# lhwright13/Hybrid-Classical-and-Reinforcement-Learning-Aircraft-Controllers

Hardware: AMD Instinct MI355X
Metric: env-steps/sec (whole node), rate-control task, batch 65536 per GPU (higher is better)
Workload: dtype f32 compute / f64 state

## Files before the change

hybrid-classical-and-reinforcement-learning-aircraft-controllers_amd/csrc/fdyn_kernels.hip:

```cpp
#include <hip/hip_runtime.h>
#include <stdint.h>
#include <math.h>
#include <string.h>
#include <stdlib.h>
#include "fdyn_core.hpp"
#include "../../include/fdyn.h"

using namespace fdyn;

#define FD_BLOCK 256
#define FD_MAX_TYPES 8
#define FD_WAVE 64

template <typename T>
__device__ __forceinline__ void stage(T* dst, const T* __restrict__ src, int n)
{
    for (int i = threadIdx.x; i < n; i += blockDim.x) dst[i] = src[i];
}

template <bool FAST>
__device__ __forceinline__ void stage_params(double* s_params, const double* __restrict__ params, int n_types)
{
    for (int i = threadIdx.x; i < n_types * FD_NP_USED; i += blockDim.x) {
        const int t = i / FD_NP_USED, k = i - t * FD_NP_USED;
// ... 443 lines not shown
            if (idx >= n_wp) { if (restart) idx = 0; else frozen = true; }
            if (!frozen) surf = waypoint_agent<G>(cfg, st, Cr, s_wps + idx * FD_NWP, xg, derive(), gdt, inner);
            return;
        }
        const G c0 = G(cmd[i]), c1 = G(cmd[n + i]), c2 = G(cmd[2 * n + i]), c3 = G(cmd[3 * n + i]);
        if (level == FD_LEVEL_ATTITUDE) {
            const bool has_yaw = c2 == c2;
            surf = attitude_agent<G>(cfg, st, Cr, c0, c1, has_yaw ? c2 : G(0), has_yaw, c3, xg, gdt, inner);
        } else if (level == FD_LEVEL_HSA) {
            surf = hsa_agent<G>(cfg, st, Cr, c0, c1, c2, xg, derive(), gdt, inner);
        } else {
            const G wp[FD_NWP] = { c0, c1, c2, c3 };
            surf = waypoint_agent<G>(cfg, st, Cr, wp, xg, derive(), gdt, inner);
        }
    };
    if constexpr (FAST) {
        FastRK f;
        f.init(x);
        outer(f.x0, [&]() { return derived_fast(f); });
    } else {
        outer(x, [&]() { return derived<S>(x); });
    }

#pragma unroll
    for (int k = 0; k < FD_NX; ++k) if (actions) xs[k * n + i] = x[k];
#pragma unroll
    for (int k = 0; k < FD_NPID; ++k) {
        pid_state[(k * FD_NPS + FD_PS_INTEGRAL) * n + i] = st[k].integral;
        pid_state[(k * FD_NPS + FD_PS_ERR_PREV) * n + i] = st[k].err_prev;
        pid_state[(k * FD_NPS + FD_PS_DFILT) * n + i] = st[k].dfilt;
    }
    if (mission) {
        wp_idx[i] = idx;
        if (reached_total) reached_total[i] += reached;
    }
    if (is_pid) {
        surf_out[FD_U_ELEVATOR * n + i] = S(surf.elevator); surf_out[FD_U_AILERON * n + i] = S(surf.aileron);
        surf_out[FD_U_RUDDER * n + i] = S(surf.rudder);
    } else if (actions) {
        surf_out[FD_U_ELEVATOR * n + i] = S(applied.elevator); surf_out[FD_U_AILERON * n + i] = S(applied.aileron);
        surf_out[FD_U_RUDDER * n + i] = S(applied.rudder);
    }
    surf_out[FD_U_THROTTLE * n + i] = S(surf.throttle);
    const float rc[4] = { float(inner.p), float(inner.q), float(inner.r), float(inner.thr) };
    if (rate_cmd_out) {
#pragma unroll
        for (int k = 0; k < 4; ++k) rate_cmd_out[k * n + i] = rc[k];
    }
    {
#pragma clang fp contract(off)
        float* o = obs_out + i * FD_OBS_DIM;
        const double mr[3] = { consts[FD_C_MAX_ROLL_RATE], consts[FD_C_MAX_PITCH_RATE], consts[FD_C_MAX_YAW_RATE] };
#pragma unroll
        for (int k = 0; k < 3; ++k) {
            const S c = clipv(S(rc[k]), -S(mr[k]), S(mr[k]));
            o[k] = float(x[9 + k]);
            o[3 + k] = float(c);
            o[6 + k] = float(c - x[9 + k]);
        }
        o[9] = float(M<S>::sqrt(x[3] * x[3] + x[4] * x[4] + x[5] * x[5]));
        o[10] = float(-x[2]);
        o[11] = float(x[6]); o[12] = float(x[7]); o[13] = float(x[8]);
#pragma unroll
        for (int k = 0; k < FD_ACT_DIM; ++k) o[14 + k] = pa[k];
    }
}

template <typename G> struct EnvConsts {
    G dt, mr0, mr1, mr2, scale;
    int max_steps, cmd_type, n_sub;
    int settle_steps;
    __device__ __forceinline__ G max_rate(int ax) const { return mr0 * G(ax == 0) + mr1 * G(ax == 1) + mr2 * G(ax == 2); }
};

template <typename G>
__device__ __forceinline__ void env_load(EnvState<G>& e, const G* __restrict__ es, int64_t n, int64_t i, bool sched = true)
{
#pragma unroll
    for (int k = 0; k < 3; ++k) {
        e.cmd[k] = es[(FD_E_CMD_P + k) * n + i];
        e.prev_err[k] = es[(FD_E_PERR_P + k) * n + i];
        e.sign_changes[k] = es[(FD_E_SIGN_P + k) * n + i];
    }
#pragma unroll
    for (int k = 0; k < 4; ++k) {
        e.prev_action[k] = es[(FD_E_PREV_AIL + k) * n + i];
        e.sched[k] = sched ? es[(FD_E_SCHED0 + k) * n + i] : G(0);
    }
    e.settle_timer = es[FD_E_SETTLE_TIMER * n + i]; e.is_settled = es[FD_E_IS_SETTLED * n + i];
    e.time = es[FD_E_TIME * n + i]; e.ep_return = es[FD_E_EP_RETURN * n + i];
}
template <typename G>
__device__ __forceinline__ void env_store(const EnvState<G>& e, G* __restrict__ es, int64_t n, int64_t i, bool sched = true)
{
#pragma unroll
    for (int k = 0; k < 3; ++k) {
        es[(FD_E_CMD_P + k) * n + i] = e.cmd[k];
        es[(FD_E_PERR_P + k) * n + i] = e.prev_err[k];
        es[(FD_E_SIGN_P + k) * n + i] = e.sign_changes[k];
    }
#pragma unroll
    for (int k = 0; k < 4; ++k) {
        es[(FD_E_PREV_AIL + k) * n + i] = e.prev_action[k];
        if (sched) es[(FD_E_SCHED0 + k) * n + i] = e.sched[k];
    }
    es[FD_E_SETTLE_TIMER * n + i] = e.settle_timer; es[FD_E_IS_SETTLED * n + i] = e.is_settled;
    es[FD_E_TIME * n + i] = e.time; es[FD_E_EP_RETURN * n + i] = e.ep_return;
}

template <typename G>
__device__ __forceinline__ void device_reset_record(uint64_t seed, uint32_t env, uint32_t episode,
                                                    const EnvConsts<G>& ec, G (&rec)[FD_NR])
{
    Philox ph;
    uint32_t r0[4], r1[4], r2[4], r3[4];
    ph.block(seed, env, episode, 0u, FD_PHX_RESET + 0, r0);
    ph.block(seed, env, episode, 0u, FD_PHX_RESET + 1, r1);
    ph.block(seed, env, episode, 0u, FD_PHX_RESET + 2, r2);
    ph.block(seed, env, episode, 0u, FD_PHX_RESET + 3, r3);
    const float d15 = 0.26179938779914943f;
    rec[FD_R_AIRSPEED] = G(15.0f + 15.0f * u01(r0[0]));
    rec[FD_R_ALTITUDE] = G(50.0f + 150.0f * u01(r0[1]));
    rec[FD_R_ROLL] = G(-d15 + 2.0f * d15 * u01(r0[2]));
    rec[FD_R_PITCH] = G(-d15 + 2.0f * d15 * u01(r0[3]));
    rec[FD_R_YAW] = G(6.283185307179586f * u01(r1[0]));
    rec[FD_R_P] = G(-0.1f + 0.2f * u01(r1[1]));
    rec[FD_R_Q] = G(-0.1f + 0.2f * u01(r1[2]));
    rec[FD_R_R] = G(-0.1f + 0.2f * u01(r1[3]));
    rec[FD_R_CMD0] = rec[FD_R_CMD1] = rec[FD_R_CMD2] = rec[FD_R_CMD3] = G(0);
    if (ec.cmd_type == FD_CMD_RANDOM_WALK) return;
    const bool sine = ec.cmd_type == FD_CMD_SINE;
    int k = sine ? 1 + int(u01(r2[0]) * 2.0f) : 1 + int(u01(r2[0]) * 3.0f);
    k = k > 3 ? 3 : k;
    const int perm = int(u01(r2[1]) * 6.0f) % 6;
    const int first = perm >> 1;
    const int o1 = first == 2 ? 0 : first + 1, o2 = first == 0 ? 2 : first - 1;
    const int second = (perm & 1) ? o2 : o1;
    const float m0 = u01(r3[0]), m1 = u01(r3[1]), m2 = u01(r3[2]);
    const G mrs[3] = { ec.mr0, ec.mr1, ec.mr2 };
    G vals[3];
#pragma unroll
    for (int a = 0; a < 3; ++a) {
        const int pos = (a == first) ? 0 : ((a == second) ? 1 : 2);
        const float um = pos == 0 ? m0 : (pos == 1 ? m1 : m2);
        float mag = (0.3f + 0.7f * um) * float(ec.scale);
        if (sine) mag *= 0.5f;
        const float sgn = (!sine && ((r2[2] >> pos) & 1u)) ? -1.0f : 1.0f;
        vals[a] = (pos < k) ? G(sgn * mag) * mrs[a] : G(0);
    }
    rec[FD_R_CMD0] = vals[0]; rec[FD_R_CMD1] = vals[1]; rec[FD_R_CMD2] = vals[2];
    if (sine) rec[FD_R_CMD3] = G(0.1f + 1.9f * u01(r2[3]));
}

template <typename G, typename E>
__device__ __forceinline__ void env_apply_reset(const G (&rec)[FD_NR], int cmd_type, G (&x)[FD_NX], EnvState<E>& e)
{
#pragma unroll
    for (int k = 0; k < FD_NX; ++k) x[k] = G(0);
    x[2] = -rec[FD_R_ALTITUDE]; x[3] = rec[FD_R_AIRSPEED];
    x[6] = rec[FD_R_ROLL]; x[7] = rec[FD_R_PITCH]; x[8] = rec[FD_R_YAW];
    x[9] = rec[FD_R_P]; x[10] = rec[FD_R_Q]; x[11] = rec[FD_R_R];
#pragma unroll
    for (int k = 0; k < 3; ++k) { e.cmd[k] = E(0); e.prev_err[k] = E(0); e.sign_changes[k] = E(0); e.prev_action[k] = E(0); }
#pragma unroll
    for (int k = 0; k < 4; ++k) e.sched[k] = E(0);
    e.prev_action[3] = E(0.5);
    if (cmd_type == FD_CMD_STEP) {
        e.cmd[0] = E(rec[FD_R_CMD0]); e.cmd[1] = E(rec[FD_R_CMD1]); e.cmd[2] = E(rec[FD_R_CMD2]);
    } else if (cmd_type == FD_CMD_RAMP || cmd_type == FD_CMD_SINE) {
        e.sched[0] = E(rec[FD_R_CMD0]); e.sched[1] = E(rec[FD_R_CMD1]); e.sched[2] = E(rec[FD_R_CMD2]); e.sched[3] = E(rec[FD_R_CMD3]);
    }
    e.settle_timer = E(0); e.is_settled = E(0); e.time = E(0); e.ep_return = E(0);
}

template <typename G, bool PREP = false>
__device__ __forceinline__ void load_env_consts(const double* __restrict__ EC, EnvConsts<G>& ec)
{
    ec.dt = G(EC[FD_EC_DT]);
    if constexpr (!PREP) {
        ec.max_steps = int(EC[FD_EC_MAX_STEPS]);
        ec.cmd_type = int(EC[FD_EC_CMD_TYPE]);
    }
    ec.scale = G(EC[FD_EC_DIFFICULTY_SCALE]);
    ec.mr0 = G(EC[FD_EC_MAX_RATE_P]); ec.mr1 = G(EC[FD_EC_MAX_RATE_Q]); ec.mr2 = G(EC[FD_EC_MAX_RATE_R]);
    if constexpr (PREP) {
        const int32_t* __restrict__ ic = reinterpret_cast<const int32_t*>(EC + FD_ECD_INTS);
        ec.max_steps = ic[0]; ec.cmd_type = ic[1]; ec.n_sub = ic[2]; ec.settle_steps = ic[3];
        return;
    }
    const double r = EC[FD_EC_DT] / EC[FD_EC_DT_PHYSICS];
    const long ns = long(r);
    ec.n_sub = ns < 1 ? 1 : int(ns);
    const double dts = EC[FD_EC_DT];
    int k = 0;
    if (dts >= 1.0e-3) { double t = 0.0; while (t < 0.2 && k < 256) { t += dts; ++k; } }
    else k = int(0.2 / dts) + 1;
    ec.settle_steps = k;
}

template <typename G>
__device__ __forceinline__ void fetch_reset_record(const double* __restrict__ pool, int pool_depth, uint64_t seed,
                                                   int64_t i, int32_t episode, const EnvConsts<G>& ec, G (&rec)[FD_NR])
{
    if (pool) {
        const double* r = pool + (i * pool_depth + (episode % pool_depth)) * FD_NR;
#pragma unroll
        for (int k = 0; k < FD_NR; ++k) rec[k] = G(r[k]);
#pragma unroll
        for (int k = 0; k < FD_NR; ++k) asm volatile("" : "+v"(rec[k]));
    } else {
        device_reset_record<G>(seed, uint32_t(i), uint32_t(episode), ec, rec);
    }
}

__device__ __forceinline__ void store_obs_tile(float* tile , const float (&o)[FD_OBS_DIM], int lane,
                                               float* __restrict__ obs_out, int64_t wave_first, int64_t n)
{
    int64_t valid = n - wave_first;
    valid = valid < 0 ? 0 : (valid < FD_WAVE ? valid : FD_WAVE);
    float* dst = obs_out + wave_first * FD_OBS_DIM;
    static_assert(FD_OBS_DIM == 18 && FD_WAVE == 64, "the full-wave path below moves 64 x 18 floats as 288 float4");
    if (valid == FD_WAVE && (reinterpret_cast<uintptr_t>(dst) & 15) == 0) {
        float2* row = reinterpret_cast<float2*>(tile + lane * FD_OBS_DIM);
#pragma unroll
        for (int k = 0; k < FD_OBS_DIM / 2; ++k) row[k] = make_float2(o[2 * k], o[2 * k + 1]);
        __builtin_amdgcn_wave_barrier();
        const float4* t4 = reinterpret_cast<const float4*>(tile);
        float4* d4 = reinterpret_cast<float4*>(dst);
#pragma unroll
        for (int j = 0; j < 4; ++j) d4[j * FD_WAVE + lane] = t4[j * FD_WAVE + lane];
        if (lane < FD_WAVE / 2) d4[4 * FD_WAVE + lane] = t4[4 * FD_WAVE + lane];
        __builtin_amdgcn_wave_barrier();
        return;
    }
#pragma unroll
    for (int k = 0; k < FD_OBS_DIM; ++k) tile[lane * (FD_OBS_DIM + 1) + k] = o[k];
    __builtin_amdgcn_wave_barrier();
#pragma unroll
    for (int k = 0; k < FD_OBS_DIM; ++k) {
        const int flat = k * FD_WAVE + lane;
        const int row = flat / FD_OBS_DIM, col = flat - row * FD_OBS_DIM;
        if (row < valid) dst[flat] = tile[row * (FD_OBS_DIM + 1) + col];
    }
    __builtin_amdgcn_wave_barrier();
}

template <typename S> __device__ __forceinline__ void dr_unpack(S*& dr, const double*& drc, S* d, const double* c) { dr = d; drc = c; }
__device__ __forceinline__ void dr_normals3(uint64_t seed, uint32_t env, uint32_t episode, uint32_t step, uint32_t word, float (&z)[3])
{
    Philox ph; uint32_t r[4];
    ph.block(seed, env, episode, step, word, r);
    const float m0 = fast::sqrt(-2.0f * __logf(u01(r[0]))), m1 = fast::sqrt(-2.0f * __logf(u01(r[2])));
    float s0, c0, s1, c1;
    fast::sincos(6.283185307179586f * u01(r[1]), s0, c0);
    fast::sincos(6.283185307179586f * u01(r[3]), s1, c1);
    z[0] = m0 * c0; z[1] = m0 * s0; z[2] = m1 * c1;
}
template <typename A, typename S>
__device__ __forceinline__ void air_velocity(const S (&x)[FD_NX], const S (&W)[3], A& ua, A& va, A& wa)
{
    A sp, cp, st, ct, sy, cy, bu, bv, bw;
    M<A>::sincos(A(x[6]), sp, cp); M<A>::sincos(A(x[7]), st, ct); M<A>::sincos(A(x[8]), sy, cy);
    body_wind<A>(sp, cp, st, ct, sy, cy, Wind<A>{ A(W[0]), A(W[1]), A(W[2]) }, bu, bv, bw);
    ua = A(x[3]) - bu; va = A(x[4]) - bv; wa = A(x[5]) - bw;
}
template <typename A, typename S>
__device__ __forceinline__ A air_speed(const S (&x)[FD_NX], const S (&W)[3])
{
    A ua, va, wa;
    air_velocity<A, S>(x, W, ua, va, wa);
    return M<A>::sqrt(ua * ua + va * va + wa * wa);
}
template <typename S>
__device__ __forceinline__ void dr_reset(uint64_t seed, uint32_t env, uint32_t episode, const double* __restrict__ drc, double dt,
                                         S* __restrict__ dr, int64_t n, int64_t i, S (&x)[FD_NX], S (&wair)[3])
{
    if (drc[FD_DC_REDRAW] != 0.0) {
        Philox ph;
        uint32_t r0[4], r1[4], r2[4];
        ph.block(seed, env, episode, 0u, FD_PHX_DR_RESET, r0);
        ph.block(seed, env, episode, 0u, FD_PHX_DR_RESET + 1, r1);
        ph.block(seed, env, episode, 0u, FD_PHX_DR_RESET + 2, r2);
        const uint32_t u[10] = { r0[0], r0[1], r0[2], r0[3], r1[0], r1[1], r1[2], r1[3], r2[0], r2[1] };
        double v[10];
#pragma unroll
        for (int k = 0; k < 10; ++k) {
            const double lo = drc[2 * k], hi = drc[2 * k + 1];
            v[k] = lo + (hi - lo) * double(u01(u[k]));
        }
        float sd, cd;
        fast::sincos(float(v[1]), sd, cd);
        float z[3];
        dr_normals3(seed, env, episode, 0u, FD_PHX_DR_GUST0, z);
        const double V0 = double(x[3]);
        const double sigma = v[3] * V0;
        const double a = exp(-dt * V0 / v[4]);
        const S row[FD_NDR] = { S(v[0] * double(cd)), S(v[0] * double(sd)), S(v[2]),
                                S(sigma * double(z[0])), S(sigma * double(z[1])), S(sigma * double(z[2])),
                                S(a), S(sigma * sqrt(1.0 - a * a)),
                                S(v[5]), S(v[6]), S(v[7]), S(v[8]), S(v[9]) };
#pragma unroll
        for (int k = 0; k < FD_NDR; ++k) dr[k * n + i] = row[k];
#pragma unroll
        for (int k = 0; k < 3; ++k) wair[k] = row[FD_DR_WIND_N + k] + row[FD_DR_GUST_N + k];
    } else {
#pragma unroll
        for (int k = 0; k < 3; ++k) wair[k] = dr[(FD_DR_WIND_N + k) * n + i] + dr[(FD_DR_GUST_N + k) * n + i];
    }
    S sp, cp, st, ct, sy, cy, bu, bv, bw;
    M<S>::sincos(x[6], sp, cp); M<S>::sincos(x[7], st, ct); M<S>::sincos(x[8], sy, cy);
    body_wind<S>(sp, cp, st, ct, sy, cy, Wind<S>{ wair[0], wair[1], wair[2] }, bu, bv, bw);
    x[3] = x[3] + bu; x[4] = x[4] + bv; x[5] = x[5] + bw;
}

template <typename S, typename E, typename... DRA>
__global__ void __launch_bounds__(FD_BLOCK)
rate_env_reset_kernel(S* __restrict__ xs, E* __restrict__ es, int32_t* __restrict__ eis, float* __restrict__ pid_state,
                      const uint8_t* __restrict__ mask, const double* __restrict__ EC, const double* __restrict__ pool,
                      int pool_depth, uint64_t seed, float* __restrict__ obs_out, int64_t n, DRA... dra)
{
    __shared__ __attribute__((aligned(16))) float s_tile[FD_BLOCK / FD_WAVE][FD_WAVE * (FD_OBS_DIM + 1)];
    constexpr bool DR = sizeof...(DRA) != 0;
    S* dr = nullptr;
    const double* drc = nullptr;
    if constexpr (DR) dr_unpack(dr, drc, dra...);
    const LaneMap lm = lane_map(n);
    const int64_t i = lm.i;
    const int lane = lm.lane, wave = threadIdx.x / FD_WAVE;
    const bool active = lm.on;
    EnvConsts<S> ec;
    load_env_consts<S>(EC, ec);
    S x[FD_NX];
    EnvState<E> e;
    float o[FD_OBS_DIM];
#pragma unroll
    for (int k = 0; k < FD_OBS_DIM; ++k) o[k] = 0.0f;
    if (active) {
        const bool doit = mask ? mask[i] != 0 : true;
        S wair[3];
        if (doit) {
            const int32_t episode = eis[FD_EI_EPISODE * n + i];
            S rec[FD_NR];
            fetch_reset_record<S>(pool, pool_depth, seed, i, episode, ec, rec);
            env_apply_reset<S, E>(rec, ec.cmd_type, x, e);
            if constexpr (DR) dr_reset<S>(seed, uint32_t(i), uint32_t(episode), drc, EC[FD_EC_DT], dr, n, i, x, wair);
#pragma unroll
            for (int k = 0; k < FD_NX; ++k) xs[k * n + i] = x[k];
            env_store<E>(e, es, n, i);
            eis[FD_EI_STEP * n + i] = 0;
            eis[FD_EI_EPISODE * n + i] = episode + 1;
            if (pid_state) for (int k = 0; k < 3 * FD_NPS; ++k) pid_state[k * n + i] = 0.0f;
        } else {
#pragma unroll
            for (int k = 0; k < FD_NX; ++k) x[k] = xs[k * n + i];
            env_load<E>(e, es, n, i);
            if constexpr (DR) {
#pragma unroll
                for (int k = 0; k < 3; ++k) wair[k] = dr[(FD_DR_WIND_N + k) * n + i] + dr[(FD_DR_GUST_N + k) * n + i];
            }
        }
        S airspeed, altitude;
        airspeed_altitude<S>(x, airspeed, altitude);
        if constexpr (DR) airspeed = air_speed<S, S>(x, wair);
        env_observation<S, S, E>(x, e, airspeed, altitude, o);
    }
    store_obs_tile(s_tile[wave], o, lane, obs_out, lm.wave_first, n);
}

#ifdef FD_PHASE_STAMPS
__device__ unsigned long long fdyn_stamps[4096 * 8];
#define FD_STAMP(K) if (threadIdx.x == 0 && blockIdx.x < 4096) fdyn_stamps[blockIdx.x * 8 + (K)] = __builtin_readcyclecounter();
#define FD_STAMP_REAL(K) if (threadIdx.x == 0 && blockIdx.x < 4096) fdyn_stamps[blockIdx.x * 8 + (K)] = wall_clock64();
extern "C" int fdyn_debug_read_stamps(unsigned long long* out, int count)
{
    return int(hipMemcpyFromSymbol(out, HIP_SYMBOL(fdyn_stamps), sizeof(unsigned long long) * size_t(count)));
}
extern "C" int fdyn_debug_read_counts(unsigned* out, int count, int clear)
{
    int rc = int(hipMemcpyFromSymbol(out, HIP_SYMBOL(fdyn_dbg_cnt), sizeof(unsigned) * size_t(count)));
    if (clear && rc == 0) {
        void* p = nullptr;
        rc = int(hipGetSymbolAddress(&p, HIP_SYMBOL(fdyn_dbg_cnt)));
        if (rc == 0) rc = int(hipMemset(p, 0, sizeof(unsigned) * 4096 * 8));
    }
    return rc;
}
#else
#define FD_STAMP(K)
#define FD_STAMP_REAL(K)
#endif

template <typename S, typename T, bool OCC2, bool PREP, typename... DRA>
__global__ void __launch_bounds__(FD_BLOCK, OCC2 ? 2 : 1)
rate_env_step_kernel(S* __restrict__ xs, typename EnvOf<S, T>::type* __restrict__ es, int32_t* __restrict__ eis,
                     const uint8_t* __restrict__ type, const double* __restrict__ params, int n_types,
                     const double* __restrict__ EC,
                     const float* __restrict__ actions ,
                     float* __restrict__ pid_state , const float* __restrict__ pid_cfg ,
                     const double* __restrict__ casc_consts , float* __restrict__ actions_out,
                     const S* __restrict__ rw_delta ,
                     const double* __restrict__ pool, int pool_depth, uint64_t seed, int auto_reset, float residual_scale,
                     float* __restrict__ obs_out , float* __restrict__ reward_f32, S* __restrict__ reward_full,
                     uint8_t* __restrict__ terminated, uint8_t* __restrict__ truncated,
                     int32_t* __restrict__ ev_count, int32_t* __restrict__ ev_count_next, int32_t* __restrict__ ev_int,
                     float* __restrict__ ev_flt, int ev_cap, int64_t n, DRA... dra)
{
    constexpr bool DR = sizeof...(DRA) != 0;
    S* dr = nullptr;
    const double* drc = nullptr;
    if constexpr (DR) dr_unpack(dr, drc, dra...);
    __shared__ double s_params[FD_MAX_TYPES * FD_NP_STAGED];
    __shared__ __attribute__((aligned(16))) float s_tile[FD_BLOCK / FD_WAVE][FD_WAVE * (FD_OBS_DIM + 1)];
    __shared__ float s_pid_cfg[3 * FD_NPC];
    __shared__ S s_consts[FD_NC];
    FD_STAMP(0)
    FD_STAMP_REAL(7)
    const LaneMap lm = lane_map(n);
    const int64_t i = lm.i;
    const int lane = lm.lane, wave = threadIdx.x / FD_WAVE;
    const bool active = lm.on;
    EnvConsts<S> ec;
    load_env_consts<S, PREP>(EC, ec);
    const bool uses_sched = ec.cmd_type == FD_CMD_RAMP || ec.cmd_type == FD_CMD_SINE;
    const bool residual_mode = actions != nullptr && residual_scale > 0.0f && pid_state != nullptr;
    const bool pid_mode = actions == nullptr || residual_mode;

    using E = typename EnvOf<S, T>::type;
    S x[FD_NX];
    EnvState<E> e;
    int32_t step = 0, episode = 0;
    int ty = 0;
    float4 av = make_float4(0.0f, 0.0f, 0.0f, 0.0f);
    S rec_pre[FD_NR];
    S wair[3] = { S(0), S(0), S(0) }, dsc[5] = { S(1), S(1), S(1), S(1), S(1) };
    const bool pre_drawn = !OCC2 && pool == nullptr && auto_reset != 0;
    constexpr bool EARLY_PARAMS = sizeof(T) == 4;
    StagedParamWords spw = { 0.0, 0.0, 1.0 };
    if constexpr (EARLY_PARAMS) spw = PREP ? stage_image_early(params, n_types) : stage_params_early(params, n_types);
    if (active) {
        episode = eis[FD_EI_EPISODE * n + i];
#pragma unroll
        for (int k = 3; k < FD_NX; ++k) x[k] = xs[k * n + i];
        if (actions) av = reinterpret_cast<const float4*>(actions)[i];
        ty = lane_type(type, i, n_types);
#pragma unroll
        for (int k = 0; k < 3; ++k) x[k] = xs[k * n + i];
        step = eis[FD_EI_STEP * n + i];
        env_load<E>(e, es, n, i, uses_sched);
        if (pre_drawn) device_reset_record<S>(seed, uint32_t(i), uint32_t(episode), ec, rec_pre);
        if constexpr (DR) {
#pragma unroll
            for (int k = 0; k < 3; ++k) wair[k] = dr[(FD_DR_WIND_N + k) * n + i] + dr[(FD_DR_GUST_N + k) * n + i];
#pragma unroll
            for (int k = 0; k < 5; ++k) dsc[k] = dr[(FD_DR_MASS_S + k) * n + i];
        }
    }
    if constexpr (PREP) {
        if constexpr (EARLY_PARAMS) stage_image_finish(s_params, spw, n_types);
        else stage(s_params, params, n_types * FD_NP_STAGED);
    } else if constexpr (EARLY_PARAMS) stage_params_finish<true>(s_params, spw, n_types);
    else stage_params<false>(s_params, params, n_types);
    if (pid_mode) {
        stage(s_pid_cfg, pid_cfg, 3 * FD_NPC);
        for (int k = threadIdx.x; k < FD_NC; k += blockDim.x) s_consts[k] = S(casc_consts[k]);
    }
    __syncthreads();

    if (ev_count_next && blockIdx.x == 0 && threadIdx.x < FD_EV_SHARDS) ev_count_next[threadIdx.x] = 0;

    float o[FD_OBS_DIM];
#pragma unroll
    for (int k = 0; k < FD_OBS_DIM; ++k) o[k] = 0.0f;
    bool done = false, term = false;
    S reward = S(0);

    if (active) {
        const double* blk = s_params + ty * FD_NP_STAGED;
        Params<T> P; P.load(blk);
        if constexpr (DR) scale_params<T>(P, double(dsc[0]), double(dsc[1]), double(dsc[2]), double(dsc[3]), double(dsc[4]));
        Limits<S> Lm; Lm.load(blk);

        float a_in[4];
        S res_bonus = S(0);
        if (!pid_mode) {
            a_in[0] = av.x; a_in[1] = av.y; a_in[2] = av.z; a_in[3] = av.w;
        } else {
            PidCfg cfg[3]; PidState st[3];
#pragma unroll
            for (int k = 0; k < 3; ++k) {
                cfg[k] = load_pid_cfg(s_pid_cfg, k);
                st[k] = PidState{ pid_state[(k * FD_NPS + 0) * n + i], pid_state[(k * FD_NPS + 1) * n + i], pid_state[(k * FD_NPS + 2) * n + i] };
            }
            const S pid_dt = s_consts[FD_C_PID_DT] > S(0) ? s_consts[FD_C_PID_DT] : ec.dt;
            const Surfaces<S> sf = rate_agent<S>(cfg, st, s_consts, S(e.cmd[0]), S(e.cmd[1]), S(e.cmd[2]), s_consts[FD_C_PID_THROTTLE], x, pid_dt);
            a_in[0] = float(sf.aileron); a_in[1] = float(sf.elevator); a_in[2] = float(sf.rudder); a_in[3] = float(sf.throttle);
#pragma unroll
            for (int k = 0; k < 3; ++k) {
                pid_state[(k * FD_NPS + 0) * n + i] = st[k].integral; pid_state[(k * FD_NPS + 1) * n + i] = st[k].err_prev;
                pid_state[(k * FD_NPS + 2) * n + i] = st[k].dfilt;
            }
            if (residual_mode) {
#pragma clang fp contract(off)
                const float rr[4] = { av.x, av.y, av.z, av.w };
#pragma unroll
                for (int k = 0; k < 4; ++k) {
                    const float c = a_in[k] + rr[k] * residual_scale;
                    const float lo = k < 3 ? -1.0f : 0.0f;
                    a_in[k] = c < lo ? lo : (c > 1.0f ? 1.0f : c);
                }
                const float mag = rr[0] * rr[0] + (rr[1] * rr[1] + rr[2] * rr[2]);
                res_bonus = S(0.05) * (S(1) - S(mag) / S(3));
            }
        }
        if (actions_out) reinterpret_cast<float4*>(actions_out)[i] = make_float4(a_in[0], a_in[1], a_in[2], a_in[3]);
        S a[4];
        a[0] = clipv(S(a_in[0]), S(-1), S(1)); a[1] = clipv(S(a_in[1]), S(-1), S(1));
        a[2] = clipv(S(a_in[2]), S(-1), S(1)); a[3] = clipv(S(a_in[3]), S(0), S(1));

        Controls<T> C;
        C.set(P, a[1], a[0], a[2], a[3]);
        const S dt_sub = ec.dt / S(ec.n_sub);
#ifdef FD_PHASE_STAMPS
        asm volatile("s_waitcnt vmcnt(0) lgkmcnt(0)" ::: "memory");
#endif
        FD_STAMP(1)
        if constexpr (DR) rk4_substeps<S, T, !OCC2, true>(P, Lm, C, x, dt_sub, ec.n_sub, Wind<T>{ T(wair[0]), T(wair[1]), T(wair[2]) });
        else rk4_substeps<S, T, !OCC2>(P, Lm, C, x, dt_sub, ec.n_sub);
        FD_STAMP(2)
        if constexpr (sizeof(E) == sizeof(S)) e.time += E(ec.dt);
        else e.time = E(S(step + 1) * ec.dt);
        step += 1;

        if (ec.cmd_type == FD_CMD_RAMP) {
            const S t = S(e.time);
            if (t < S(3)) {
                const S alpha = t / S(3);
#pragma unroll
                for (int k = 0; k < 3; ++k) e.cmd[k] = E((S(1) - alpha) * S(0) + alpha * S(e.sched[k]));
            } else {
#pragma unroll
                for (int k = 0; k < 3; ++k) e.cmd[k] = e.sched[k];
            }
        } else if (ec.cmd_type == FD_CMD_RANDOM_WALK) {
            S delta[3];
            if (rw_delta) {
#pragma unroll
                for (int k = 0; k < 3; ++k) delta[k] = rw_delta[k * n + i];
            } else {
                Philox ph; uint32_t r[4];
                ph.block(seed, uint32_t(i), uint32_t(episode), uint32_t(step), FD_PHX_RANDOM_WALK, r);
                const float m0 = sqrtf(-2.0f * logf(u01(r[0]))), m1 = sqrtf(-2.0f * logf(u01(r[2])));
                const float n0 = m0 * cosf(6.283185307f * u01(r[1])), n1 = m0 * sinf(6.283185307f * u01(r[1]));
                const float n2 = m1 * cosf(6.283185307f * u01(r[3]));
                const S sd = S(0.1) * M<S>::sqrt(ec.dt) * ec.scale;
                delta[0] = S(n0) * sd * ec.mr0; delta[1] = S(n1) * sd * ec.mr1; delta[2] = S(n2) * sd * ec.mr2;
            }
#pragma unroll
            for (int k = 0; k < 3; ++k) e.cmd[k] = E(clipv(S(e.cmd[k]) + delta[k], -ec.max_rate(k), ec.max_rate(k)));
        } else if (ec.cmd_type == FD_CMD_SINE) {
            const S sn = M<S>::sin(S(2.0 * FD_PI) * S(e.sched[3]) * S(e.time));
#pragma unroll
            for (int k = 0; k < 3; ++k) e.cmd[k] = E(S(e.sched[k]) * sn);
        }

        if constexpr (DR) {
            float z[3];
            dr_normals3(seed, uint32_t(i), uint32_t(episode), uint32_t(step), FD_PHX_GUST, z);
            const S ga = dr[FD_DR_GUST_A * n + i], gb = dr[FD_DR_GUST_B * n + i];
#pragma unroll
            for (int k = 0; k < 3; ++k) {
                const S g = ga * dr[(FD_DR_GUST_N + k) * n + i] + gb * S(z[k]);
                dr[(FD_DR_GUST_N + k) * n + i] = g;
                wair[k] = dr[(FD_DR_WIND_N + k) * n + i] + g;
            }
        }

        using A = typename GlueOf<S, T>::type;
        const A u_ = A(x[3]), v_ = A(x[4]), w_ = A(x[5]), roll_ = A(x[6]), pitch_ = A(x[7]);
        A airspeed = M<A>::sqrt(u_ * u_ + v_ * v_ + w_ * w_);
        if constexpr (DR) airspeed = air_speed<A, S>(x, wair);
        const A altitude = -A(x[2]);
        const A err[3] = { A(e.cmd[0]) - A(x[9]), A(e.cmd[1]) - A(x[10]), A(e.cmd[2]) - A(x[11]) };
        const A aa[4] = { A(a[0]), A(a[1]), A(a[2]), A(a[3]) };
        A rew = env_reward<E, A>(e, err, aa, airspeed, altitude, roll_, pitch_, ec.dt, ec.settle_steps);
#pragma unroll
        for (int k = 0; k < 4; ++k) e.prev_action[k] = E(a[k]);
        term = (altitude < A(5)) || (M<A>::abs(roll_) > deg2rad<A>(120.0)) || (M<A>::abs(pitch_) > deg2rad<A>(80.0)) ||
               (airspeed < A(8));
        const bool trunc = step >= ec.max_steps;
        if (term && !trunc) rew += A(-100);
        reward = S(rew) + res_bonus;
        e.ep_return += E(reward);
        done = term || trunc;
        env_observation<S, A, E>(x, e, airspeed, altitude, o);
        if (reward_f32) reward_f32[i] = float(reward);
        if (reward_full) reward_full[i] = reward;
        terminated[i] = term ? 1 : 0;
        truncated[i] = trunc ? 1 : 0;
    }

    FD_STAMP(3)
    const unsigned long long done_mask = __ballot(done);
    const bool compact = done_mask != 0ull && ev_count != nullptr;
    int base = 0, prefix = 0;
    const int shard = int(blockIdx.x) & (FD_EV_SHARDS - 1), cap_s = ev_cap / FD_EV_SHARDS;
    if (compact) {
        const int n_done = __popcll(done_mask);
        prefix = __builtin_amdgcn_mbcnt_hi(uint32_t(done_mask >> 32), __builtin_amdgcn_mbcnt_lo(uint32_t(done_mask), 0u));
        const int leader = __ffsll((long long)done_mask) - 1;
        if (lane == leader) {
            int cnt = shard;
            asm volatile("" : "+v"(cnt));
            base = atomicAdd(ev_count + cnt, n_done);
        }
    }
    float o_term[FD_OBS_DIM];
#pragma unroll
    for (int k = 0; k < FD_OBS_DIM; ++k) o_term[k] = o[k];
    const float ret_term = done ? float(e.ep_return) : 0.0f;
    const int32_t len_term = step;

    if (active) {
        if (done && auto_reset) {
            S rec[FD_NR];
            if (pre_drawn) {
#pragma unroll
                for (int k = 0; k < FD_NR; ++k) rec[k] = rec_pre[k];
            } else {
                fetch_reset_record<S>(pool, pool_depth, seed, i, episode, ec, rec);
            }
            env_apply_reset<S, E>(rec, ec.cmd_type, x, e);
            if constexpr (DR) dr_reset<S>(seed, uint32_t(i), uint32_t(episode), drc, EC[FD_EC_DT], dr, n, i, x, wair);
            step = 0;
            episode += 1;
            using A0 = typename GlueOf<S, T>::type;
            A0 xa[FD_NX];
#pragma unroll
            for (int k = 0; k < FD_NX; ++k) xa[k] = A0(x[k]);
            A0 airspeed, altitude;
            airspeed_altitude<A0>(xa, airspeed, altitude);
            if constexpr (DR) airspeed = air_speed<A0, S>(x, wair);
            env_observation<S, A0, E>(x, e, airspeed, altitude, o);
            if (pid_mode) for (int k = 0; k < 3 * FD_NPS; ++k) pid_state[k * n + i] = 0.0f;
        }
#pragma unroll
        for (int k = 0; k < FD_NX; ++k) xs[k * n + i] = x[k];
        env_store<E>(e, es, n, i, uses_sched);
        eis[FD_EI_STEP * n + i] = step;
        eis[FD_EI_EPISODE * n + i] = episode;
        if (compact) {
            asm volatile("" : "+v"(base) : : "memory");
            const int leader = __ffsll((long long)done_mask) - 1;
            base = __shfl(base, leader, FD_WAVE);
            const int local = base + prefix;
            if (done && local < cap_s) {
                const int slot = shard * cap_s + local;
                ev_int[slot * FD_EV_NI + FD_EV_ENV] = int32_t(i);
                ev_int[slot * FD_EV_NI + FD_EV_LENGTH] = len_term;
                ev_int[slot * FD_EV_NI + FD_EV_TERMINATED] = term ? 1 : 0;
                ev_flt[slot * FD_EV_NF] = ret_term;
#pragma unroll
                for (int k = 0; k < FD_OBS_DIM; ++k) ev_flt[slot * FD_EV_NF + 1 + k] = o_term[k];
            }
        }
    }
    FD_STAMP(4)
    store_obs_tile(s_tile[wave], o, lane, obs_out, lm.wave_first, n);
    FD_STAMP(5)
#ifdef FD_PHASE_STAMPS
    asm volatile("s_waitcnt vmcnt(0)" ::: "memory");
#endif
    FD_STAMP_REAL(6)
}

static_assert(FD_NIMG == FD_IMG_PARAMS + FD_MAX_TYPES * FD_NP_STAGED && FD_ECD_INTS + 2 <= FD_IMG_PARAMS, "fdyn_layout.h: image sections");
template <bool FAST>
__global__ void __launch_bounds__(FD_BLOCK)
rate_env_image_kernel(const double* __restrict__ params, int n_types, const double* __restrict__ EC, double* __restrict__ image)
{
    double* blocks = image + FD_IMG_PARAMS;
    for (int i = threadIdx.x; i < FD_MAX_TYPES * FD_NP_STAGED; i += blockDim.x) {
        const int t = i / FD_NP_STAGED, k = i - t * FD_NP_STAGED;
        blocks[i] = (t < n_types && k < FD_NP_USED) ? params[t * FD_NP + k] : 0.0;
    }
    for (int k = threadIdx.x; k < FD_IMG_PARAMS; k += blockDim.x) if (k < FD_ECD_INTS || k >= FD_ECD_INTS + 2) image[FD_IMG_EC + k] = k < FD_NEC ? EC[k] : 0.0;
    __syncthreads();
    constexpr int NDL = Params<double>::FD_ND_LANES;
    if (int(threadIdx.x) < n_types * NDL) {
        const int t = threadIdx.x / NDL;
        Params<double>::derive_lane<FAST>(threadIdx.x - t * NDL, params + t * FD_NP, blocks + t * FD_NP_STAGED);
    }
    if (threadIdx.x == FD_BLOCK - 1) {
        EnvConsts<double> ec;
        load_env_consts<double>(EC, ec);
        int32_t* ic = reinterpret_cast<int32_t*>(image + FD_IMG_EC + FD_ECD_INTS);
        ic[0] = ec.max_steps; ic[1] = ec.cmd_type; ic[2] = ec.n_sub; ic[3] = ec.settle_steps;
    }
}

static int g_simds = 0;
static int simd_count()
{
    if (!g_simds) {
        int dev = 0; hipDeviceProp_t p;
        g_simds = (hipGetDevice(&dev) == hipSuccess && hipGetDeviceProperties(&p, dev) == hipSuccess) ? p.multiProcessorCount * 4 : 1024;
    }
    return g_simds;
}

template <typename K, typename... A>
static int launch(K kernel, int64_t n, void* stream, A... args)
{
    hipLaunchKernelGGL(kernel, dim3(unsigned((n + FD_BLOCK - 1) / FD_BLOCK)), dim3(FD_BLOCK), 0, (hipStream_t)stream, args...);
    return int(hipGetLastError());
}

#define FD_CHECK_COMMON(n, n_types)                                       \
    if ((n) < 0 || (n) > (int64_t(1) << 31) - FD_BLOCK) return FDYN_ERR_BAD_SIZE;   \
    if ((n_types) < 1 || (n_types) > FD_MAX_TYPES) return FDYN_ERR_BAD_TYPES;       \
    if ((n) == 0) return FDYN_OK;

static inline bool bad_dt(double dt) { return !(dt > 1e-6) || dt > 1.0; }

#define FD_ENV_RESET_PARAMS(S, E)                                                                            \
    S* x, E* e, int32_t* ei, float* pid_state, const uint8_t* mask, const double* env_consts, const double* pool, \
    int pool_depth, uint64_t seed, float* obs_out, int64_t n
#define FD_ENV_RESET_ARGS x, e, ei, pid_state, mask, env_consts, pool, pool_depth, seed, obs_out, n
#define FD_ENV_STEP_PARAMS(S, E)                                                                             \
    S* x, E* e, int32_t* ei, const uint8_t* type, const double* params, int n_types, const double* env_consts, \
    const float* actions, float* pid_state, const float* pid_cfg, const double* casc_consts, float* actions_out, \
    const S* rw_delta, const double* pool, int pool_depth, uint64_t seed, int auto_reset, float residual_scale, \
    float* obs_out, float* reward_f32, S* reward_full, uint8_t* terminated, uint8_t* truncated, int32_t* ev_count, \
    int32_t* ev_count_next, int32_t* ev_int, float* ev_flt, int ev_cap, int64_t n
#define FD_ENV_STEP_ARGS                                                                                     \
    x, e, ei, type, params, n_types, env_consts, actions, pid_state, pid_cfg, casc_consts, actions_out, rw_delta, pool, \
    pool_depth, seed, auto_reset, residual_scale, obs_out, reward_f32, reward_full, terminated, truncated, ev_count, \
    ev_count_next, ev_int, ev_flt, ev_cap, n

template <typename S, typename E, typename... DRA>
static int env_reset(FD_ENV_RESET_PARAMS(S, E), void* stream, DRA... dra)
{
    if ((... || !dra)) return FDYN_ERR_NULL;
    FD_CHECK_COMMON(n, 1)
    if (pool && pool_depth < 1) return FDYN_ERR_BAD_SIZE;
    return launch(rate_env_reset_kernel<S, E, DRA...>, n, stream, FD_ENV_RESET_ARGS, dra...);
}

template <typename S, typename E, typename T, bool PREP, typename... DRA>
static int env_step(FD_ENV_STEP_PARAMS(S, E), void* stream, DRA... dra)
{
    if ((... || !dra)) return FDYN_ERR_NULL;
    FD_CHECK_COMMON(n, n_types)
    if (pool && pool_depth < 1) return FDYN_ERR_BAD_SIZE;
    if ((!actions || residual_scale > 0.0f) && !(pid_state && pid_cfg && casc_consts)) return FDYN_ERR_NULL;
    if (!obs_out || !terminated || !truncated || !env_consts) return FDYN_ERR_NULL;
    if (ev_count && (!ev_int || !ev_flt)) return FDYN_ERR_NULL;
    if (ev_count && (ev_cap < FD_EV_SHARDS || ev_cap % FD_EV_SHARDS != 0)) return FDYN_ERR_BAD_SIZE;
    constexpr bool FP32 = sizeof(T) == 4;
    const bool occ2 = FP32 && n > int64_t(simd_count()) * FD_WAVE;
    return launch(occ2 ? rate_env_step_kernel<S, T, FP32, PREP, DRA...> : rate_env_step_kernel<S, T, false, PREP, DRA...>, n, stream,
                  FD_ENV_STEP_ARGS, dra...);
}

extern "C" {

int fdyn_abi_version(void) { return FDYN_ABI_VERSION; }

int fdyn_num_substeps(double dt, double dt_physics)
{
    const double r = dt / dt_physics;
    const long n = long(r);
    return n < 1 ? 1 : int(n);
}

int64_t fdyn_event_capacity(int64_t n)
{
    const int64_t blocks = (n + FD_BLOCK - 1) / FD_BLOCK;
    return FD_EV_SHARDS * ((blocks + FD_EV_SHARDS - 1) / FD_EV_SHARDS) * FD_BLOCK;
}

int fdyn_device_info(int* cu_count, int* wave_size, char* arch, int arch_len)
{
    hipDeviceProp_t p;
    int dev = 0;
    hipError_t e = hipGetDevice(&dev);
    if (e != hipSuccess) return int(e);
    e = hipGetDeviceProperties(&p, dev);
    if (e != hipSuccess) return int(e);
    if (cu_count) *cu_count = p.multiProcessorCount;
    if (wave_size) *wave_size = p.warpSize;
    if (arch && arch_len > 0) { strncpy(arch, p.gcnArchName, arch_len - 1); arch[arch_len - 1] = 0; }
    return FDYN_OK;
}

#define FD_DEFINE_SIXDOF(NAME, S, T)                                                                         \
    int NAME(S* x, const S* u, const uint8_t* type, const double* params, int n_types, int64_t n, double dt, \
             int n_sub, S* derived_out, void* stream)                                                        \
    {                                                                                                        \
        FD_CHECK_COMMON(n, n_types)                                                                          \
        if (n_sub < 1) return FDYN_ERR_BAD_SIZE;                                                             \
        const double dt_sub = dt / n_sub;                                                                    \
        if (bad_dt(dt_sub)) return FDYN_ERR_BAD_DT;                                                          \
        return launch(sixdof_step_kernel<S, T>, n, stream, x, u, type, params, n_types, n, S(dt_sub), n_sub, derived_out); \
    }
FD_DEFINE_SIXDOF(fdyn_sixdof_step_f64, double, double)
FD_DEFINE_SIXDOF(fdyn_sixdof_step_mixed, double, float)
FD_DEFINE_SIXDOF(fdyn_sixdof_step_f32, float, float)

int fdyn_derived_f64(const double* x, int64_t n, double* out, void* stream)
{
    FD_CHECK_COMMON(n, 1)
    return launch(derived_kernel<double>, n, stream, x, n, out);
}
int fdyn_derived_f32(const float* x, int64_t n, float* out, void* stream)
{
    FD_CHECK_COMMON(n, 1)
    return launch(derived_kernel<float>, n, stream, x, n, out);
}

int fdyn_pid_compute_batch(const float* cfg, int cfg_per_lane, float* state, const float* setpoint,
// ... 105 lines not shown
```

Before: 1.776 billion.

## Issue state stores early and move obs tile store inside active branch

Computes the termination condition right after integration and writes the post-reset state vector to global memory early, so those stores overlap the reward and observation work. For full waves the observation tile store now happens inside the active region before the env-state stores, and the event compaction moves inside the active branch. This reorders the global writes to hide store latency, at the cost of extra live registers (a copy of the state plus the reset record) and some duplicated reset-record fetching logic. It also adds a scratch script that counts memory ops in the compiled kernel.

```diff
diff --git a/hybrid-classical-and-reinforcement-learning-aircraft-controllers_amd/csrc/fdyn_kernels.hip b/hybrid-classical-and-reinforcement-learning-aircraft-controllers_amd/csrc/fdyn_kernels.hip
--- a/hybrid-classical-and-reinforcement-learning-aircraft-controllers_amd/csrc/fdyn_kernels.hip
+++ b/hybrid-classical-and-reinforcement-learning-aircraft-controllers_amd/csrc/fdyn_kernels.hip
@@ -619,14 +619,19 @@
     if (sine) rec[FD_R_CMD3] = G(0.1f + 1.9f * u01(r2[3]));
 }
 
-template <typename G, typename E>
-__device__ __forceinline__ void env_apply_reset(const G (&rec)[FD_NR], int cmd_type, G (&x)[FD_NX], EnvState<E>& e)
+template <typename G>
+__device__ __forceinline__ void state_apply_reset(const G (&rec)[FD_NR], G (&x)[FD_NX])
 {
 #pragma unroll
     for (int k = 0; k < FD_NX; ++k) x[k] = G(0);
     x[2] = -rec[FD_R_ALTITUDE]; x[3] = rec[FD_R_AIRSPEED];
     x[6] = rec[FD_R_ROLL]; x[7] = rec[FD_R_PITCH]; x[8] = rec[FD_R_YAW];
     x[9] = rec[FD_R_P]; x[10] = rec[FD_R_Q]; x[11] = rec[FD_R_R];
+}
+template <typename G, typename E>
+__device__ __forceinline__ void env_apply_reset(const G (&rec)[FD_NR], int cmd_type, G (&x)[FD_NX], EnvState<E>& e)
+{
+    state_apply_reset<G>(rec, x);
 #pragma unroll
     for (int k = 0; k < 3; ++k) { e.cmd[k] = E(0); e.prev_err[k] = E(0); e.sign_changes[k] = E(0); e.prev_action[k] = E(0); }
 #pragma unroll
@@ -886,6 +891,7 @@
     const int64_t i = lm.i;
     const int lane = lm.lane, wave = threadIdx.x / FD_WAVE;
     const bool active = lm.on;
+    const bool full_wave = int64_t(blockIdx.x) * FD_BLOCK + __builtin_amdgcn_readfirstlane(int(threadIdx.x) & ~(FD_WAVE - 1)) + FD_WAVE <= n;
     EnvConsts<S> ec;
     load_env_consts<S, PREP>(EC, ec);
     const bool uses_sched = ec.cmd_type == FD_CMD_RAMP || ec.cmd_type == FD_CMD_SINE;
@@ -940,6 +946,8 @@
     for (int k = 0; k < FD_OBS_DIM; ++k) o[k] = 0.0f;
     bool done = false, term = false;
     S reward = S(0);
+    constexpr bool EARLY_STORES = !DR;
+    S rec[FD_NR];
 
     if (active) {
         const double* blk = s_params + ty * FD_NP_STAGED;
@@ -998,6 +1006,38 @@
         else e.time = E(S(step + 1) * ec.dt);
         step += 1;
 
+        using A = typename GlueOf<S, T>::type;
+        A airspeed = A(0), altitude = A(0), roll_ = A(0), pitch_ = A(0);
+        bool trunc = false;
+        auto flight_condition = [&]() {
+            const A u_ = A(x[3]), v_ = A(x[4]), w_ = A(x[5]);
+            roll_ = A(x[6]); pitch_ = A(x[7]);
+            airspeed = M<A>::sqrt(u_ * u_ + v_ * v_ + w_ * w_);
+            if constexpr (DR) airspeed = air_speed<A, S>(x, wair);
+            altitude = -A(x[2]);
+            term = (altitude < A(5)) || (M<A>::abs(roll_) > deg2rad<A>(120.0)) || (M<A>::abs(pitch_) > deg2rad<A>(80.0)) ||
+                   (airspeed < A(8));
+            trunc = step >= ec.max_steps;
+            done = term || trunc;
+        };
+        if constexpr (EARLY_STORES) {
+            flight_condition();
+            S xn[FD_NX];
+#pragma unroll
+            for (int k = 0; k < FD_NX; ++k) xn[k] = x[k];
+            if (done && auto_reset) {
+                if (pre_drawn) {
+#pragma unroll
+                    for (int k = 0; k < FD_NR; ++k) rec[k] = rec_pre[k];
+                } else {
+                    fetch_reset_record<S>(pool, pool_depth, seed, i, episode, ec, rec);
+                }
+                state_apply_reset<S>(rec, xn);
+            }
+#pragma unroll
+            for (int k = 0; k < FD_NX; ++k) xs[k * n + i] = xn[k];
+        }
+
         if (ec.cmd_type == FD_CMD_RAMP) {
             const S t = S(e.time);
             if (t < S(3)) {
@@ -1042,59 +1082,50 @@
             }
         }
 
-        using A = typename GlueOf<S, T>::type;
-        const A u_ = A(x[3]), v_ = A(x[4]), w_ = A(x[5]), roll_ = A(x[6]), pitch_ = A(x[7]);
-        A airspeed = M<A>::sqrt(u_ * u_ + v_ * v_ + w_ * w_);
-        if constexpr (DR) airspeed = air_speed<A, S>(x, wair);
-        const A altitude = -A(x[2]);
+        if constexpr (!EARLY_STORES) flight_condition();
         const A err[3] = { A(e.cmd[0]) - A(x[9]), A(e.cmd[1]) - A(x[10]), A(e.cmd[2]) - A(x[11]) };
         const A aa[4] = { A(a[0]), A(a[1]), A(a[2]), A(a[3]) };
         A rew = env_reward<E, A>(e, err, aa, airspeed, altitude, roll_, pitch_, ec.dt, ec.settle_steps);
 #pragma unroll
         for (int k = 0; k < 4; ++k) e.prev_action[k] = E(a[k]);
-        term = (altitude < A(5)) || (M<A>::abs(roll_) > deg2rad<A>(120.0)) || (M<A>::abs(pitch_) > deg2rad<A>(80.0)) ||
-               (airspeed < A(8));
-        const bool trunc = step >= ec.max_steps;
         if (term && !trunc) rew += A(-100);
         reward = S(rew) + res_bonus;
         e.ep_return += E(reward);
-        done = term || trunc;
         env_observation<S, A, E>(x, e, airspeed, altitude, o);
         if (reward_f32) reward_f32[i] = float(reward);
         if (reward_full) reward_full[i] = reward;
         terminated[i] = term ? 1 : 0;
         truncated[i] = trunc ? 1 : 0;
-    }
-
-    FD_STAMP(3)
-    const unsigned long long done_mask = __ballot(done);
-    const bool compact = done_mask != 0ull && ev_count != nullptr;
-    int base = 0, prefix = 0;
-    const int shard = int(blockIdx.x) & (FD_EV_SHARDS - 1), cap_s = ev_cap / FD_EV_SHARDS;
-    if (compact) {
-        const int n_done = __popcll(done_mask);
-        prefix = __builtin_amdgcn_mbcnt_hi(uint32_t(done_mask >> 32), __builtin_amdgcn_mbcnt_lo(uint32_t(done_mask), 0u));
-        const int leader = __ffsll((long long)done_mask) - 1;
-        if (lane == leader) {
-            int cnt = shard;
-            asm volatile("" : "+v"(cnt));
-            base = atomicAdd(ev_count + cnt, n_done);
-        }
-    }
-    float o_term[FD_OBS_DIM];
-#pragma unroll
-    for (int k = 0; k < FD_OBS_DIM; ++k) o_term[k] = o[k];
-    const float ret_term = done ? float(e.ep_return) : 0.0f;
-    const int32_t len_term = step;
-
-    if (active) {
+
+        FD_STAMP(3)
+        const unsigned long long done_mask = __ballot(done);
+        const bool compact = done_mask != 0ull && ev_count != nullptr;
+        int base = 0, prefix = 0;
+        const int shard = int(blockIdx.x) & (FD_EV_SHARDS - 1), cap_s = ev_cap / FD_EV_SHARDS;
+        if (compact) {
+            const int n_done = __popcll(done_mask);
+            prefix = __builtin_amdgcn_mbcnt_hi(uint32_t(done_mask >> 32), __builtin_amdgcn_mbcnt_lo(uint32_t(done_mask), 0u));
+            const int leader = __ffsll((long long)done_mask) - 1;
+            if (lane == leader) {
+                int cnt = shard;
+                asm volatile("" : "+v"(cnt));
+                base = atomicAdd(ev_count + cnt, n_done);
+            }
+        }
+        float o_term[FD_OBS_DIM];
+#pragma unroll
+        for (int k = 0; k < FD_OBS_DIM; ++k) o_term[k] = o[k];
+        const float ret_term = done ? float(e.ep_return) : 0.0f;
+        const int32_t len_term = step;
+
         if (done && auto_reset) {
-            S rec[FD_NR];
-            if (pre_drawn) {
-#pragma unroll
-                for (int k = 0; k < FD_NR; ++k) rec[k] = rec_pre[k];
-            } else {
-                fetch_reset_record<S>(pool, pool_depth, seed, i, episode, ec, rec);
+            if constexpr (!EARLY_STORES) {
+                if (pre_drawn) {
+#pragma unroll
+                    for (int k = 0; k < FD_NR; ++k) rec[k] = rec_pre[k];
+                } else {
+                    fetch_reset_record<S>(pool, pool_depth, seed, i, episode, ec, rec);
+                }
             }
             env_apply_reset<S, E>(rec, ec.cmd_type, x, e);
             if constexpr (DR) dr_reset<S>(seed, uint32_t(i), uint32_t(episode), drc, EC[FD_EC_DT], dr, n, i, x, wair);
@@ -1110,13 +1141,17 @@
             env_observation<S, A0, E>(x, e, airspeed, altitude, o);
             if (pid_mode) for (int k = 0; k < 3 * FD_NPS; ++k) pid_state[k * n + i] = 0.0f;
         }
-#pragma unroll
-        for (int k = 0; k < FD_NX; ++k) xs[k * n + i] = x[k];
+        FD_STAMP(4)
+        if (full_wave) store_obs_tile(s_tile[wave], o, lane, obs_out, lm.wave_first, n);
+        if constexpr (!EARLY_STORES) {
+#pragma unroll
+            for (int k = 0; k < FD_NX; ++k) xs[k * n + i] = x[k];
+        }
         env_store<E>(e, es, n, i, uses_sched);
         eis[FD_EI_STEP * n + i] = step;
         eis[FD_EI_EPISODE * n + i] = episode;
+        asm volatile("" : "+v"(base) : : "memory");
         if (compact) {
-            asm volatile("" : "+v"(base) : : "memory");
             const int leader = __ffsll((long long)done_mask) - 1;
             base = __shfl(base, leader, FD_WAVE);
             const int local = base + prefix;
@@ -1131,8 +1166,7 @@
             }
         }
     }
-    FD_STAMP(4)
-    store_obs_tile(s_tile[wave], o, lane, obs_out, lm.wave_first, n);
+    if (!full_wave) store_obs_tile(s_tile[wave], o, lane, obs_out, lm.wave_first, n);
     FD_STAMP(5)
 #ifdef FD_PHASE_STAMPS
     asm volatile("s_waitcnt vmcnt(0)" ::: "memory");
diff --git a/scratch/count_vmem.py b/scratch/count_vmem.py
--- /dev/null
+++ b/scratch/count_vmem.py
@@ -0,0 +1,50 @@
+import collections, os, re, subprocess, sys, tempfile
+REPO = os.path.dirname(os.path.dirname(os.path.abspath(__file__)))
+src = os.path.join(REPO, "hybrid-classical-and-reinforcement-learning-aircraft-controllers_amd", "csrc", "fdyn_kernels.hip")
+flags = [a for a in sys.argv[1:] if a.startswith("-D")]
+md = "--md" in sys.argv
+asm = next((a for a in sys.argv[1:] if a.endswith(".s")), None)
+if asm is None:
+    asm = os.path.join(tempfile.mkdtemp(), "fdyn_kernels.s")
+    subprocess.check_call(["/opt/rocm/bin/hipcc", "--offload-arch=gfx950", "-O3", "-std=c++17", "--cuda-device-only", "-S", *flags, src,
+                           "-o", asm], stderr=subprocess.DEVNULL)
+lines = open(asm).read().split("\n")
+WIDTH = {"": 4, "dword": 4, "dwordx2": 8, "dwordx3": 12, "dwordx4": 16, "ubyte": 1, "sbyte": 1, "byte": 1, "ushort": 2, "short": 2}
+rows, name, body = {}, None, None
+for l in lines:
+    if re.match(r"_Z\w*rate_env_\w*:", l):
+        name, body = l.split(":")[0], collections.Counter()
+    elif name and body is not None:
+        m = re.match(r"\s*(global|buffer|flat)_(load|store|atomic)_(\w+)", l)
+        if m:
+            body[(m.group(2), m.group(3))] += 1
+        if "s_endpgm" in l:
+            rows[name] = {"ops": body}
+            body = None
+    m = re.match(r"\s*\.amdhsa_kernel (\S+)", l)
+    if m:
+        cur = m.group(1)
+    elif ".amdhsa_private_segment_fixed_size" in l and cur in rows:
+        rows[cur]["priv"] = int(l.split()[-1])
+    elif ".amdhsa_next_free_vgpr" in l and cur in rows:
+        rows[cur]["vgpr"] = int(l.split()[-1])
+def short(nm):
+    t = {"d": "double", "f": "float"}
+    m = re.match(r"_Z\d+rate_env_step_kernelI([df])([df])Lb([01])ELb([01])EJ(E?)", nm)
+    if m:
+        return (f"step<{t[m.group(1)]},{t[m.group(2)]},OCC2={m.group(3)},PREP={m.group(4)}" + ("" if m.group(5) else ",DR") + ">")
+    m = re.match(r"_Z\d+rate_env_reset_kernelI([df])([df])J(E?)", nm)
+    if m:
+        return f"reset<{t[m.group(1)]},{t[m.group(2)]}" + ("" if m.group(3) else ",DR") + ">"
+    return nm[:60]
+hdr = ["kernel", "ld b8", "ld x1", "ld x2", "ld x4", "st b8", "st x1", "st x2", "st x4", "atomic", "private B", "VGPR"]
+if md:
+    print("| " + " | ".join(hdr) + " |\n|" + "---|" * len(hdr))
+for nm, r in rows.items():
+    c = r["ops"]
+    def cnt(kind, names):
+        return sum(v for (k, w), v in c.items() if k == kind and w in names)
+    vals = [short(nm), cnt("load", ("ubyte", "sbyte")), cnt("load", ("dword",)), cnt("load", ("dwordx2",)), cnt("load", ("dwordx4",)),
+            cnt("store", ("byte",)), cnt("store", ("dword",)), cnt("store", ("dwordx2",)), cnt("store", ("dwordx4",)),
+            sum(v for (k, w), v in c.items() if k == "atomic"), r.get("priv", -1), r.get("vgpr", -1)]
+    print(("| " + " | ".join(str(v) for v in vals) + " |") if md else "  ".join(f"{v!s:>5}" if j else f"{v!s:70s}" for j, v in enumerate(vals)))
```

After: 1.780 billion (median of 4 runs). Within noise of the previous version (+0.2%).
